# kfjahnke/envutil

Measured on AMD Instinct MI355X. Metric: Mpix/s reprojected (16K lat/lon->cubemap, b-spline-3), higher is better.
Workload: dtype f32

## Files before the change

### envutil_amd/csrc/eu_render5.h

```cpp
#define EU5_WAVES 4
#ifndef EU5_TEXELS
#define EU5_TEXELS 576
#endif
#ifndef EU5_OCC
#define EU5_OCC 4
#endif
#ifndef EU5_UNIT_ROWS
#define EU5_UNIT_ROWS 4
#endif

typedef const __attribute__((address_space(3))) eu4_f4 *eu5_l4ptr;

template <int NCH, int DEG>
__device__ __forceinline__ void eu5_taps(eu_lptr lt, int a, int b, int pitch, const eu_f2 *wx, const eu_f2 *wy,
                                         eu_f2 tx, eu_f2 ty, eu_f2 &rga, eu_f2 &bxa, eu_f2 &rgb, eu_f2 &bxb)
{
  constexpr int order = DEG + 1;
  if constexpr (DEG == 1) {
    const eu_f2 wl0 = 1.0f - tx, wr0 = tx, wl1 = 1.0f - ty, wr1 = ty;
    const eu4_f4 a00 = *(eu5_l4ptr)(lt + a), a01 = *(eu5_l4ptr)(lt + a + 4);
    const eu4_f4 a10 = *(eu5_l4ptr)(lt + a + pitch), a11 = *(eu5_l4ptr)(lt + a + pitch + 4);
    const eu4_f4 b00 = *(eu5_l4ptr)(lt + b), b01 = *(eu5_l4ptr)(lt + b + 4);
    const eu4_f4 b10 = *(eu5_l4ptr)(lt + b + pitch), b11 = *(eu5_l4ptr)(lt + b + pitch + 4);
    {
      const eu_f2 l0 = { wl0.x, wl0.x }, r0 = { wr0.x, wr0.x }, l1 = { wl1.x, wl1.x }, r1 = { wr1.x, wr1.x };
      eu_f2 s = a00.xy * l0; s = s + a01.xy * r0; s = s * l1;
      eu_f2 u = a10.xy * l0; u = u + a11.xy * r0; rga = s + u * r1;
      s = a00.zw * l0; s = s + a01.zw * r0; s = s * l1;
      u = a10.zw * l0; u = u + a11.zw * r0; bxa = s + u * r1;
    }
    {
      const eu_f2 l0 = { wl0.y, wl0.y }, r0 = { wr0.y, wr0.y }, l1 = { wl1.y, wl1.y }, r1 = { wr1.y, wr1.y };
      eu_f2 s = b00.xy * l0; s = s + b01.xy * r0; s = s * l1;
      eu_f2 u = b10.xy * l0; u = u + b11.xy * r0; rgb = s + u * r1;
      s = b00.zw * l0; s = s + b01.zw * r0; s = s * l1;
      u = b10.zw * l0; u = u + b11.zw * r0; bxb = s + u * r1;
    }
  } else {
#pragma unroll
    for (int j = 0; j < order; j++) {
      eu4_f4 ta[order], tb[order];
#pragma unroll
      for (int i = 0; i < order; i++) {
        ta[i] = *(eu5_l4ptr)(lt + a + j * pitch + 4 * i);
        tb[i] = *(eu5_l4ptr)(lt + b + j * pitch + 4 * i);
      }
      const eu_f2 w0a = { wx[0].x, wx[0].x }, w0b = { wx[0].y, wx[0].y };
      eu_f2 ra = ta[0].xy * w0a, qa = ta[0].zw * w0a, rb = tb[0].xy * w0b, qb = tb[0].zw * w0b;
#pragma unroll
      for (int i = 1; i < order; i++) {
        const eu_f2 wa = { wx[i].x, wx[i].x }, wb = { wx[i].y, wx[i].y };
        ra = EU_MAD2(wa, ta[i].xy, ra); qa = EU_MAD2(wa, ta[i].zw, qa);
        rb = EU_MAD2(wb, tb[i].xy, rb); qb = EU_MAD2(wb, tb[i].zw, qb);
      }
      const eu_f2 ya = { wy[j].x, wy[j].x }, yb = { wy[j].y, wy[j].y };
      if (j == 0) { rga = ra * ya; bxa = qa * ya; rgb = rb * yb; bxb = qb * yb; }
      else { rga = EU_MAD2(ra, ya, rga); bxa = EU_MAD2(qa, ya, bxa); rgb = EU_MAD2(rb, yb, rgb); bxb = EU_MAD2(qb, yb, bxb); }
    }
  }
}

__device__ __forceinline__ void eu5_box_reduce(int &q0, int &q1, int &q2, int &q3, int &h0, int &h1, int &h2, int &h3)
{
#define EU5_RED(ctrl)                                        \
  "v_min_i32_dpp %0, %0, %0 " ctrl "\n\t"                    \
  "v_min_i32_dpp %1, %1, %1 " ctrl "\n\t"                    \
  "v_max_i32_dpp %2, %2, %2 " ctrl "\n\t"                    \
  "v_max_i32_dpp %3, %3, %3 " ctrl "\n\t"
  asm("s_nop 1\n\t"
      EU5_RED("row_shr:1 row_mask:0xf bank_mask:0xf")
      EU5_RED("row_shr:2 row_mask:0xf bank_mask:0xf")
      EU5_RED("row_shr:4 row_mask:0xf bank_mask:0xf")
      EU5_RED("row_shr:8 row_mask:0xf bank_mask:0xf")
      "v_mov_b32 %4, %0\n\tv_mov_b32 %5, %1\n\tv_mov_b32 %6, %2\n\tv_mov_b32 %7, %3\n\t"
      "v_min_i32_dpp %4, %0, %4 row_bcast:15 row_mask:0xa bank_mask:0xf\n\t"
      "v_min_i32_dpp %5, %1, %5 row_bcast:15 row_mask:0xa bank_mask:0xf\n\t"
      "v_max_i32_dpp %6, %2, %6 row_bcast:15 row_mask:0xa bank_mask:0xf\n\t"
      "v_max_i32_dpp %7, %3, %7 row_bcast:15 row_mask:0xa bank_mask:0xf\n\t"
      "s_nop 0"
      : "+v"(q0), "+v"(q1), "+v"(q2), "+v"(q3), "=&v"(h0), "=&v"(h1), "=&v"(h2), "=&v"(h3));
#undef EU5_RED
}

struct eu5_box { int mnx, mny, mxx, mxy; };

struct eu5_divtab_t { unsigned v[65]; };
static constexpr eu5_divtab_t eu5_make_divtab()
{
  eu5_divtab_t t = {};
  t.v[0] = 0;
  for (unsigned w = 1; w <= 64; w++) t.v[w] = ((65536u + w - 1) / w) | ((64u / w) << 24);
  return t;
}
__constant__ const eu5_divtab_t eu5_divtab = eu5_make_divtab();

__device__ __forceinline__ eu5_box eu5_box_at(int a, int b, int c, int d, int lane)
{
  eu5_box r;
  r.mnx = __builtin_amdgcn_readlane(a, lane); r.mny = __builtin_amdgcn_readlane(b, lane);
  r.mxx = __builtin_amdgcn_readlane(c, lane); r.mxy = __builtin_amdgcn_readlane(d, lane);
  return r;
}
__device__ __forceinline__ eu5_box eu5_box_join(const eu5_box &a, const eu5_box &b)
{
  eu5_box r = { min(a.mnx, b.mnx), min(a.mny, b.mny), max(a.mxx, b.mxx), max(a.mxy, b.mxy) };
  return r;
}
template <int ORDER>
__device__ __forceinline__ int eu5_box_fits(const eu5_box &b)
{
  if (b.mnx == INT_MAX) return -1;
  const unsigned bw = (unsigned)b.mxx - (unsigned)b.mnx + ORDER, bh = (unsigned)b.mxy - (unsigned)b.mny + ORDER;
  return bw <= 64u && bh <= (unsigned)EU5_TEXELS && bw * bh <= (unsigned)EU5_TEXELS;
}

__device__ __forceinline__ eu_f2 eu5_gate2(eu_f2 c, int kind, float lower, float upper)
{
  if (kind == 0) {
    eu_f2 r = c;
    r = eu_sel2(c < lower, (eu_f2){ lower, lower }, r);
    r = eu_sel2(c > upper, (eu_f2){ upper, upper }, r);
    return r;
  }
  eu_f2 cc = c - lower;
  if (kind == 1) cc = eu_abs2(cc);
  return cc + lower;
}

__device__ __forceinline__ int eu5_out_of_range3(float a, float b, float c)
{
  const float hi = __builtin_fmaxf(__builtin_fmaxf(__builtin_fabsf(a), __builtin_fabsf(b)), __builtin_fabsf(c));
  const float lo = __builtin_fminf(__builtin_fminf(__builtin_fabsf(a), __builtin_fabsf(b)), __builtin_fabsf(c));
  return (hi <= 0x1p40f && lo >= 0x1p-40f) ? 0 : -1;
}

struct eu5_tab8 { eu_f2 c0; float A0, A1, A2, B0, B1, B2; };

template <bool FAST>
__device__ __forceinline__ void eu5_load8(const eu_render_params &p, int tile_y, int x0, int lane, eu5_tab8 &T)
{
  const int pr = lane & 3, rw = (lane >> 2) & 7, hf = lane >> 5;
  const int y = p.row_begin + tile_y * EU4_TH + rw;
  const int yc = y < p.row_end ? y : p.row_end - 1;
  const float *rt = p.row + (long long)(FAST ? yc : eu_frame_row(yc, p.band_shift, p.band_count, p.band_index)) * EU_ROW_FLOATS;
  const int xa = x0 + 8 * hf + 2 * pr, xb = xa + 1;
  const int xac = xa < p.width ? xa : p.width - 1, xbc = xb < p.width ? xb : p.width - 1;
  T.A0 = rt[0]; T.A1 = rt[1]; T.A2 = rt[2]; T.B0 = rt[3]; T.B1 = rt[4]; T.B2 = rt[5];
  T.c0 = (eu_f2){ p.col[xac], p.col[xbc] };
}

struct eu5_co8 {
  eu_f2 tx, ty;
  int ixa, ixb, iya, iyb;
  eu_i2 ok;
};

template <int DEG>
__device__ __forceinline__ void eu5_coords8(const eu_src_dev &s, const float *atab, const eu5_tab8 &T, eu5_co8 &c)
{
  eu_i2 big0 = { 0, 0 }, big1 = { 0, 0 };
  const eu_f2 c0 = T.c0;
  const eu_f2 rx = T.B0 * c0 + T.A0, ry = T.B1 * c0 + T.A1, rz = T.B2 * c0 + T.A2;
  const eu_i2 ok = { ~eu5_out_of_range3(rx.x, ry.x, rz.x), ~eu5_out_of_range3(rx.y, ry.y, rz.y) };
  const eu_f2 q2 = rx * rx + rz * rz;
  const eu_f2 qs = eu_sqrt2_safe(q2);
  const eu_f2 lat = eu_atan2f_2_lean(ry, qs, atab, 1, big0);
  const eu_f2 lon = eu_atan2f_2_lean(rx, rz, atab, 0, big1);
  c.ok = ok & ~(big0 | big1);
  eu_f2 i0 = { (float)((double)lon.x - s.tex_x0), (float)((double)lon.y - s.tex_x0) };
  if (s.cdiv_ok) i0 = eu_div2_const(i0, s.ext_w, s.rcp_ext_w);
  else i0 = eu_div2_rr(i0, s.ext_w, eu_rcp_refined(s.ext_w));
  i0 = i0 * s.total_w; i0 = i0 - .5f;
  const eu_f2 sx = i0 - s.win_x_off;
  const eu_f2 gx = eu5_gate2(sx, s.gate0, s.lower0, s.upper0);
  eu_f2 fx;
  if constexpr (DEG & 1) fx = (eu_f2){ floorf(gx.x), floorf(gx.y) };
  else fx = (eu_f2){ roundf(gx.x), roundf(gx.y) };
  c.tx = gx - fx;
  c.ixa = (int)fx.x; c.ixb = (int)fx.y;
  eu_f2 i1 = { (float)((double)lat.x - s.tex_y0), (float)((double)lat.y - s.tex_y0) };
  if (s.cdiv_ok) i1 = eu_div2_const(i1, s.ext_h, s.rcp_ext_h);
  else i1 = eu_div2_rr(i1, s.ext_h, eu_rcp_refined(s.ext_h));
  i1 = i1 * s.total_h; i1 = i1 - .5f;
  const eu_f2 sy = i1 - s.win_y_off;
  c.ty = eu5_gate2(sy, s.gate1, s.lower1, s.upper1);
}

template <int DEG>
__device__ __forceinline__ void eu5_split_y(eu5_co8 &c)
{
  const eu_f2 gy = c.ty;
  eu_f2 fy;
  if constexpr (DEG & 1) fy = (eu_f2){ floorf(gy.x), floorf(gy.y) };
  else fy = (eu_f2){ roundf(gy.x), roundf(gy.y) };
  c.ty = gy - fy;
  c.iya = (int)fy.x; c.iyb = (int)fy.y;
}

struct eu5_boxes {
  int q0, q1, q2, q3, h0, h1, h2, h3;
  eu5_box full;
  int npass;
  bool clean;
};

template <int DEG, bool GATES>
__device__ __forceinline__ void eu5_box_stage(int gate0, int gate1, float upper0, float upper1, eu_i2 hit, eu_i2 ok,
                                              int ixa, int ixb, int iya, int iyb, eu5_boxes &b)
{
  constexpr int order = DEG + 1;
  int q0 = INT_MAX, q1 = INT_MAX, q2 = INT_MIN, q3 = INT_MIN, h0, h1, h2, h3;
// ... 313 lines not shown
__device__ __forceinline__ void eu5_stage(const eu_src_dev &s, const eu5_box &bx, unsigned lds_tile, int lane)
{
  constexpr int order = DEG + 1;
  const int ibw = bx.mxx - bx.mnx + order, ibh = bx.mxy - bx.mny + order;
  const unsigned tv = eu5_divtab.v[ibw];
  const int k = (int)(tv >> 24);
  const unsigned r = ((unsigned)lane * (tv & 0x1ffffu)) >> 16, c = (unsigned)lane - r * (unsigned)ibw;
  const int bx0 = bx.mnx - DEG / 2, by0 = bx.mny - DEG / 2;
  const unsigned pitchb = (unsigned)(s.es1 * 4);
  const unsigned voff = r * pitchb + c * (NCH * 4u);
  const char *const sb0 = (const char *)(s.base + ((long long)by0 * s.es1 + (long long)bx0 * NCH));
  const unsigned long long step = (unsigned long long)k * pitchb;
  const unsigned dstep = (unsigned)(k * ibw) * 16u;
  if ((int)r < k) {
    const char *sb = sb0;
    unsigned dst = lds_tile;
#pragma unroll 1
    for (int left = ibh; left >= k; left -= k) { eu4_dma_row(dst, voff, sb); sb += step; dst += dstep; }
  }
  if ((int)r < ibh % k) {
    const int full = ibh / k;
    eu4_dma_row(lds_tile + (unsigned)full * dstep, voff, sb0 + (unsigned long long)full * step);
  }
}

#define EU5_BT_RECS 4
#define EU5_BT_WORK 8
#define EU5_WAIT_VM0 0x0F70
typedef unsigned eu5_u3 __attribute__((ext_vector_type(3)));
typedef unsigned eu5_u4 __attribute__((ext_vector_type(4)));
typedef int eu5_i4 __attribute__((ext_vector_type(4)));
typedef const __attribute__((address_space(4))) eu5_i4 *eu5_crec;

__device__ __forceinline__ int eu5_bt_pack(const eu5_box &b, int w3, int c)
{
  if (c == 2) return b.mnx == INT_MAX ? -1 : (int)(((unsigned)b.mxx - (unsigned)b.mnx) | (((unsigned)b.mxy - (unsigned)b.mny) << 16));
  return c == 0 ? b.mnx : c == 1 ? b.mny : w3;
}

template <int DEG>
__global__ __launch_bounds__(256) void eu5_boxplan_kernel(const eu_render_params p, const float *atab_g, const int *l2_rows,
                                                          int tiles16, int ntiles, int *tab)
{
  __shared__ __attribute__((aligned(16))) float atab[768];
  const int lane = threadIdx.x & 63;
  const int wave = __builtin_amdgcn_readfirstlane(threadIdx.x >> 6);
  if (wave == 0) {
#pragma unroll
    for (int i = 0; i < 3; i++)
      __builtin_amdgcn_global_load_lds((eu4_gbl_void)(atab_g + i * 256 + lane * 4), (eu4_lds_void)(atab + i * 256), 16, 0, 0);
    asm volatile("s_waitcnt vmcnt(0)" ::: "memory");
  }
  __syncthreads();
  const int g = (int)blockIdx.x * 4 + wave;
  if (g >= ntiles) return;
  const int slot = g / tiles16, tcol = g - slot * tiles16;
  const int tile_y = __builtin_amdgcn_readfirstlane(l2_rows[slot]);
  const int x0 = tcol * EU4_TW;
  const eu_src_dev &s = p.src;
  const int pr = lane & 3, rw = (lane >> 2) & 7, hf = lane >> 5;
  const int y = p.row_begin + tile_y * EU4_TH + rw;
  const bool yin = y < p.row_end;
  const int xa = x0 + 8 * hf + 2 * pr, xb = xa + 1;
  const bool va = yin && xa < p.width, vb = yin && xb < p.width;
  eu5_tab8 T;
  eu5_load8<true>(p, tile_y, x0, lane, T);
  eu5_co8 c;
  eu5_coords8<DEG>(s, atab, T, c);
  eu5_split_y<DEG>(c);
  const eu_i2 hit = { va ? -1 : 0, vb ? -1 : 0 };
  eu5_boxes B;
  eu5_box_stage<DEG, true>(s.gate0, s.gate1, s.upper0, s.upper1, hit, c.ok, c.ixa, c.ixb, c.iya, c.iyb, B);
  const int cls = (B.npass < 0 || (B.npass > 0 && !B.clean)) ? EU5_BT_WORK : B.npass;
  eu5_box r[EU5_BT_RECS] = { B.full, B.full, B.full, B.full };
  if (B.npass == 2) { r[0] = eu5_box_at(B.h0, B.h1, B.h2, B.h3, 31); r[1] = eu5_box_at(B.h0, B.h1, B.h2, B.h3, 63); }
  if (B.npass == 4) {
#pragma unroll
    for (int k = 0; k < 4; k++) r[k] = eu5_box_at(B.q0, B.q1, B.q2, B.q3, 15 + 16 * k);
  }
  int v = 0;
#pragma unroll
  for (int k = 0; k < EU5_BT_RECS; k++) {
#pragma unroll
    for (int i = 0; i < 4; i++)
      if (lane == 4 * k + i) v = eu5_bt_pack(r[k], k == 0 ? cls : 0, i);
  }
  if (lane < 4 * EU5_BT_RECS) tab[(size_t)g * (4 * EU5_BT_RECS) + lane] = v;
}

template <int NCH, int DEG>
__device__ __forceinline__ void eu5_tile_bt(const eu_render_params &p, const eu4_plan &w, const float *atab, float *wtile,
                                            int tile_y, int x0, int lane, const eu5_tab8 &T, eu5_i4 R, eu5_crec rec,
                                            bool have_n, int ty_n, int x0_n, eu5_tab8 &Tn)
{
  constexpr int order = DEG + 1;
  const eu_src_dev &s = p.src;
#ifdef EU5_STAMPS
  unsigned long long st_[8] = { 0, 0, 0, 0, 0, 0, 0, 0 };
#endif
  EU5_STAMP(0);
  const int cls = R.w;
  if (cls & EU5_BT_WORK) {
    if (lane == 0) {
      const int id = tile_y * w.tiles16 + x0 / EU4_TW;
      const int sh = eu4_shard_of(id);
      const int slot = atomicAdd(p.wl + EU4_WL_SHARD(sh), 1);
      p.wl[EU4_WL_ENTRIES + (size_t)slot * EU4_SHARDS + sh] = id;
    }
    if (have_n) eu5_load8<true>(p, ty_n, x0_n, lane, Tn);
    __builtin_amdgcn_s_waitcnt(EU5_WAIT_VM0);
    return;
  }
  const int npass = cls & 7;
  const unsigned lds_tile = (unsigned)(unsigned long long)(eu4_lds_void)wtile;
  eu5_tab8 Tl = T;
  asm volatile("" : "+v"(Tl.c0), "+v"(Tl.A0), "+v"(Tl.A1), "+v"(Tl.A2), "+v"(Tl.B0), "+v"(Tl.B1), "+v"(Tl.B2));
  eu5_box bx = { R.x, R.y, R.x + (R.z & 0xffff), R.y + (R.z >> 16) };
  bool some = npass > 0 && R.z >= 0;
  if (some) eu5_stage<NCH, DEG>(s, bx, lds_tile, lane);
  const int pr = lane & 3, rw = (lane >> 2) & 7, hf = lane >> 5;
  const int y = p.row_begin + tile_y * EU4_TH + rw;
  const bool yin = y < p.row_end;
  const int xa = x0 + 8 * hf + 2 * pr, xb = xa + 1;
  const bool va = yin && xa < p.width, vb = yin && xb < p.width;
  eu_f2 rga = { 0.0f, 0.0f }, bxa = { 0.0f, 0.0f }, rgb = { 0.0f, 0.0f }, bxb = { 0.0f, 0.0f };
  if (npass > 0) {
    eu5_co8 c;
    eu5_coords8<DEG>(s, atab, Tl, c);
    eu5_split_y<DEG>(c);
#ifdef EU5_STAMPS
    asm volatile("" : : "v"(c.iya), "v"(c.iyb), "v"(c.ixa), "v"(c.ixb));
#endif
    EU5_STAMP(2);
#ifdef EU5_STAMPS
    st_[3] = st_[2];
#endif
    eu_f2 wx[order], wy[order];
    if constexpr (DEG >= 2) {
      eu_weights2<DEG>(s.wm, c.ty, wy);
      eu_weights2<DEG>(s.wm, c.tx, wx);
    }
    const int grp = npass == 1 ? 0 : npass == 2 ? hf : (lane >> 4);
#pragma unroll 1
    for (int pi = 0; pi < npass; pi++) {
      eu5_i4 Rn = { 0, 0, -1, 0 };
      if (pi + 1 < npass) Rn = rec[pi + 1];
      if (some) {
        if (pi > 0) eu5_stage<NCH, DEG>(s, bx, lds_tile, lane);
        const int ibw = bx.mxx - bx.mnx + order;
        const bool mine = grp == pi;
        const int oa = (mine && va) ? ((c.iya - bx.mny) * ibw + (c.ixa - bx.mnx)) * 4 : 0;
        const int ob = (mine && vb) ? ((c.iyb - bx.mny) * ibw + (c.ixb - bx.mnx)) * 4 : 0;
        if (pi == 0) EU5_STAMP(4);
        asm volatile("s_waitcnt vmcnt(0)" ::: "memory");
        if (pi == 0) EU5_STAMP(5);
        if (mine) eu5_taps<NCH, DEG>((eu_lptr)wtile, oa, ob, ibw * 4, wx, wy, c.tx, c.ty, rga, bxa, rgb, bxb);
      }
      bx = (eu5_box){ Rn.x, Rn.y, Rn.x + (Rn.z & 0xffff), Rn.y + (Rn.z >> 16) };
      some = Rn.z >= 0;
    }
  }
#ifdef EU5_STAMPS
  asm volatile("" : : "v"(rga), "v"(bxa), "v"(rgb), "v"(bxb));
#endif
  EU5_STAMP(6);
  float qa[4] = { rga.x, rga.y, bxa.x, bxa.y }, qb[4] = { rgb.x, rgb.y, bxb.x, bxb.y };
  if (have_n) eu5_load8<true>(p, ty_n, x0_n, lane, Tn);
  __builtin_amdgcn_sched_barrier(0);
  {
    float *const base = p.out + (long long)(tile_y * EU4_TH) * p.out_stride + (long long)x0 * NCH;
    const __amdgpu_buffer_rsrc_t rs = __builtin_amdgcn_make_buffer_rsrc(base, 0, 0x80000000u, 0x00027000);
    const unsigned off = ((unsigned)rw * (unsigned)p.out_stride + (unsigned)((8 * hf + 2 * pr) * NCH)) * 4u;
    const unsigned oa = va ? off : 0xfffff000u, ob = vb ? oa + NCH * 4u : 0xfffff000u;
    if constexpr (NCH == 3) {
      __builtin_amdgcn_raw_buffer_store_b96((eu5_u3){ __float_as_uint(qa[0]), __float_as_uint(qa[1]), __float_as_uint(qa[2]) }, rs, (int)oa, 0, 0);
      __builtin_amdgcn_raw_buffer_store_b96((eu5_u3){ __float_as_uint(qb[0]), __float_as_uint(qb[1]), __float_as_uint(qb[2]) }, rs, (int)ob, 0, 0);
    } else {
      __builtin_amdgcn_raw_buffer_store_b128((eu5_u4){ __float_as_uint(qa[0]), __float_as_uint(qa[1]), __float_as_uint(qa[2]), __float_as_uint(qa[3]) }, rs, (int)oa, 0, 0);
      __builtin_amdgcn_raw_buffer_store_b128((eu5_u4){ __float_as_uint(qb[0]), __float_as_uint(qb[1]), __float_as_uint(qb[2]), __float_as_uint(qb[3]) }, rs, (int)ob, 0, 0);
    }
  }
  EU5_STAMP(7);
#ifdef EU5_STAMPS
  if (lane == 0 && w.stamps) {
    unsigned long long *o = w.stamps + ((size_t)tile_y * w.tiles16 + x0 / EU4_TW) * 8;
    st_[1] = (unsigned long long)(npass + 1);
#pragma unroll
    for (int k = 0; k < 8; k++) o[k] = st_[k];
  }
#endif
}

struct eu5_tab16 {
  eu4_f4 a0, a1, b0, b1;
  eu_f2 c0;
  float A1A, B1A, A1B, B1B;
};

__device__ __forceinline__ void eu5_load16(const eu_render_params &p, const float *ct, int tile_y, int x0, int lane, eu5_tab16 &T)
{
  const int pr = lane & 3, rw = (lane >> 2) & 7, hf = lane >> 5;
  const int yA = p.row_begin + tile_y * EU4_TH + rw, yB = yA + EU4_TH;
  const int ycA = yA < p.row_end ? yA : p.row_end - 1, ycB = yB < p.row_end ? yB : p.row_end - 1;
  const float *rtA = p.row + (long long)ycA * EU_ROW_FLOATS, *rtB = p.row + (long long)ycB * EU_ROW_FLOATS;
  const int xa = x0 + 8 * hf + 2 * pr, xb = xa + 1;
  const int xac = xa < p.width ? xa : p.width - 1, xbc = xb < p.width ? xb : p.width - 1;
  const eu4_f4 *ea = (const eu4_f4 *)(ct + (size_t)xac * EU4_COL_FLOATS);
  const eu4_f4 *eb = (const eu4_f4 *)(ct + (size_t)xbc * EU4_COL_FLOATS);
  T.a0 = ea[0]; T.a1 = ea[1]; T.b0 = eb[0]; T.b1 = eb[1];
  T.A1A = rtA[1]; T.B1A = rtA[4]; T.A1B = rtB[1]; T.B1B = rtB[4];
  T.c0 = (eu_f2){ p.col[xac], p.col[xbc] };
}

typedef const __attribute__((address_space(4))) int *eu5_cint;

__device__ __forceinline__ void eu5_load_cols(const float *ct, int xa, int xb, eu5_tab16 &T)
{
  const eu4_f4 *ea = (const eu4_f4 *)(ct + (size_t)xa * EU4_COL_FLOATS);
  const eu4_f4 *eb = (const eu4_f4 *)(ct + (size_t)xb * EU4_COL_FLOATS);
  T.a0 = ea[0]; T.a1 = ea[1]; T.b0 = eb[0]; T.b1 = eb[1];
}

__device__ __forceinline__ void eu5_y_reduce(int &mn, int &mx)
{
#define EU5_RED2(ctrl)                                       \
  "v_min_i32_dpp %0, %0, %0 " ctrl "\n\t"                    \
  "v_max_i32_dpp %1, %1, %1 " ctrl "\n\t"                    \
  "s_nop 1\n\t"
  asm("s_nop 1\n\t"
      EU5_RED2("row_shr:1 row_mask:0xf bank_mask:0xf")
      EU5_RED2("row_shr:2 row_mask:0xf bank_mask:0xf")
      EU5_RED2("row_shr:4 row_mask:0xf bank_mask:0xf")
      EU5_RED2("row_shr:8 row_mask:0xf bank_mask:0xf")
      EU5_RED2("row_bcast:15 row_mask:0xa bank_mask:0xf")
      EU5_RED2("row_bcast:31 row_mask:0xc bank_mask:0xf")
      : "+v"(mn), "+v"(mx));
#undef EU5_RED2
  mn = __builtin_amdgcn_readlane(mn, 63); mx = __builtin_amdgcn_readlane(mx, 63);
}

template <int NCH, int DEG>
__device__ __forceinline__ void eu5_group16(const eu_render_params &p, const eu4_plan &w, const float *atab, float *wtile,
                                            eu5_tab16 &T, eu5_cint ent, int n, int m0, int plan0, int tcol, int lane0,
                                            bool have_n, int m_n, int plan_n, int tcol_n)
{
  constexpr int order = DEG + 1;
  const eu_src_dev &s = p.src;
#ifdef EU5_STAMPS
  unsigned st_[8] = { 0, 0, 0, 0, 0, 0, 0, 0 };
#endif
  EU5_STAMP32(0);
  const eu5_cint xt = (eu5_cint)w.xtab;
  int xmn = xt[2 * (plan0 * w.tiles16 + tcol)], xmx = xt[2 * (plan0 * w.tiles16 + tcol) + 1];
  int iyAa, iyAb, iyBa, iyBb, bad, mny = INT_MAX, mxy = INT_MIN;
  eu_f2 tyA, tyB;
  bool off;
  {
    int lane = lane0;
    asm volatile("" : "+v"(lane));
    const int pr = lane & 3, rw = (lane >> 2) & 7, hf = lane >> 5;
    const int yA = p.row_begin + 2 * m0 * EU4_TH + rw, yB = yA + EU4_TH;
    const bool yinA = yA < p.row_end, yinB = yB < p.row_end;
    const int xa = tcol * EU4_TW + 8 * hf + 2 * pr, xb = xa + 1;
    const bool vxa = xa < p.width, vxb = xb < p.width;
    const eu_f2 c0 = T.c0;
    const eu_f2 ryA = T.B1A * c0 + T.A1A, ryB = T.B1B * c0 + T.A1B;
    const eu_f2 qs = { T.a1.z, T.b1.z };
    eu_i2 bigA = { 0, 0 }, bigB = { 0, 0 };
    bad = eu5_out_of_range3(ryA.x, qs.x, ryB.x) | eu5_out_of_range3(ryA.y, qs.y, ryB.y);
    const eu_f2 latA = eu_atan2f_2_lean(ryA, qs, atab, 1, bigA);
    const eu_f2 latB = eu_atan2f_2_lean(ryB, qs, atab, 1, bigB);
    bad |= bigA.x | bigA.y | bigB.x | bigB.y;
    const float rr = s.cdiv_ok ? 0.0f : __int_as_float(__builtin_amdgcn_readfirstlane(__float_as_int(eu_rcp_refined(s.ext_h))));
    eu_f2 iA = { (float)((double)latA.x - s.tex_y0), (float)((double)latA.y - s.tex_y0) };
    eu_f2 iB = { (float)((double)latB.x - s.tex_y0), (float)((double)latB.y - s.tex_y0) };
    if (s.cdiv_ok) { iA = eu_div2_const(iA, s.ext_h, s.rcp_ext_h); iB = eu_div2_const(iB, s.ext_h, s.rcp_ext_h); }
    else { iA = eu_div2_rr(iA, s.ext_h, rr); iB = eu_div2_rr(iB, s.ext_h, rr); }
    iA = iA * s.total_h; iA = iA - .5f; iB = iB * s.total_h; iB = iB - .5f;
    const eu_f2 gyA = eu5_gate2(iA - s.win_y_off, s.gate1, s.lower1, s.upper1);
    const eu_f2 gyB = eu5_gate2(iB - s.win_y_off, s.gate1, s.lower1, s.upper1);
    eu_f2 fyA, fyB;
    if constexpr (DEG & 1) { fyA = (eu_f2){ floorf(gyA.x), floorf(gyA.y) }; fyB = (eu_f2){ floorf(gyB.x), floorf(gyB.y) }; }
    else { fyA = (eu_f2){ roundf(gyA.x), roundf(gyA.y) }; fyB = (eu_f2){ roundf(gyB.x), roundf(gyB.y) }; }
    tyA = gyA - fyA; tyB = gyB - fyB;
    iyAa = (int)fyA.x; iyAb = (int)fyA.y; iyBa = (int)fyB.x; iyBb = (int)fyB.y;
#ifdef EU5_STAMPS
    asm volatile("" : : "v"(iyAa), "v"(iyAb), "v"(iyBa), "v"(iyBb));
#endif
    EU5_STAMP32(2);
    const bool hAa = yinA && vxa, hAb = yinA && vxb, hBa = yinB && vxa, hBb = yinB && vxb;
    int q1 = INT_MAX, q3 = INT_MIN;
    if (hAa) { q1 = iyAa; q3 = iyAa; }
    if (hAb) { q1 = min(q1, iyAb); q3 = max(q3, iyAb); }
    if (hBa) { q1 = min(q1, iyBa); q3 = max(q3, iyBa); }
    if (hBb) { q1 = min(q1, iyBb); q3 = max(q3, iyBb); }
    eu5_y_reduce(q1, q3);
    mny = q1; mxy = q3;
    off = __ballot(bad != 0 && (hAa || hAb || hBa || hBb)) != 0ull;
  }
  EU5_STAMP32(3);
  int mk = m0, pk = plan0;
#pragma unroll 1
  for (int k = 0; k < n; k++) {
    int lane = lane0;
    asm volatile("" : "+v"(lane));
    const int pr = lane & 3, rw = (lane >> 2) & 7, hf = lane >> 5;
    const bool mir = (pk & EU_SHARE_MIRROR) != 0;
    const int tc = mir ? w.tiles16 - 1 - tcol : tcol;
    int mk_n = 0, pk_n = 0;
    if (k + 1 < n) { mk_n = ent[2 * k + 4]; pk_n = ent[2 * k + 5]; }
#ifdef EU5_STAMPS
    if (k > 0) { EU5_STAMP32(0); st_[2] = st_[0]; st_[3] = st_[0]; }
#endif
    eu5_box bx = { xmn, mny, xmx, mxy };
    bool fast = !off && xmn != INT_MAX && mny != INT_MAX;
    if (fast) {
      const int cw = __builtin_amdgcn_readfirstlane((int)(s.upper0 + 0.5f)), ch = __builtin_amdgcn_readfirstlane((int)(s.upper1 + 0.5f));
      if (s.gate0 == 2 && bx.mnx < 0) fast = false;
      if (s.gate0 != 0 && bx.mxx >= cw - 1) fast = false;
      if (s.gate1 == 2 && bx.mny < 0) fast = false;
      if (s.gate1 != 0 && bx.mxy >= ch - 1) fast = false;
      if (eu5_box_fits<order>(bx) != 1) fast = false;
    }
    const int xl = 8 * hf + 2 * pr;
    const int xa = mir ? p.width - 1 - (tcol * EU4_TW + xl) : tc * EU4_TW + xl, xb = mir ? xa - 1 : xa + 1;
    const int yA = p.row_begin + 2 * mk * EU4_TH + rw, yB = yA + EU4_TH;
    const bool yinA = yA < p.row_end, yinB = yB < p.row_end;
    const int ycA = yinA ? yA : p.row_end - 1, ycB = yinB ? yB : p.row_end - 1;
    const bool vxa = xa < p.width, vxb = xb < p.width;
    const bool hAa = yinA && vxa, hAb = yinA && vxb, hBa = yinB && vxa, hBb = yinB && vxb;
    eu_f2 rga = { 0.0f, 0.0f }, bxa = { 0.0f, 0.0f }, rgb = { 0.0f, 0.0f }, bxb = { 0.0f, 0.0f };
    if (fast) eu5_stage<NCH, DEG>(s, bx, (unsigned)(unsigned long long)(eu4_lds_void)wtile, lane);
    const bool mir_n = (pk_n & EU_SHARE_MIRROR) != 0;
    const int plan_k = pk_n & (EU_SHARE_MIRROR - 1);
    const int tc_k = mir_n ? w.tiles16 - 1 - tcol : tcol;
    int xmn_n = INT_MAX, xmx_n = INT_MIN;
    if (k + 1 < n) { xmn_n = xt[2 * (plan_k * w.tiles16 + tc_k)]; xmx_n = xt[2 * (plan_k * w.tiles16 + tc_k) + 1]; }
    if (fast) {
      eu_f2 wx[order], wyA[order], wyB[order];
      const int ixa = __float_as_int(T.a0.x), ixb = __float_as_int(T.b0.x);
      const eu_f2 tx = { T.a0.y, T.b0.y };
      if constexpr (DEG >= 2) {
        wx[0] = (eu_f2){ T.a0.z, T.b0.z }; wx[1] = (eu_f2){ T.a0.w, T.b0.w }; wx[2] = (eu_f2){ T.a1.x, T.b1.x };
        if constexpr (DEG == 3) wx[3] = (eu_f2){ T.a1.y, T.b1.y };
        eu_weights2<DEG>(s.wm, tyA, wyA); eu_weights2<DEG>(s.wm, tyB, wyB);
      }
      const int ibw = bx.mxx - bx.mnx + order;
      const int oAa = hAa ? ((iyAa - bx.mny) * ibw + (ixa - bx.mnx)) * 4 : 0, oAb = hAb ? ((iyAb - bx.mny) * ibw + (ixb - bx.mnx)) * 4 : 0;
      const int oBa = hBa ? ((iyBa - bx.mny) * ibw + (ixa - bx.mnx)) * 4 : 0, oBb = hBb ? ((iyBb - bx.mny) * ibw + (ixb - bx.mnx)) * 4 : 0;
      asm volatile("s_waitcnt vmcnt(0)" ::: "memory");
      __builtin_amdgcn_sched_barrier(0);
      eu5_taps<NCH, DEG>((eu_lptr)wtile, oAa, oAb, ibw * 4, wx, wyA, tx, tyA, rga, bxa, rgb, bxb);
      asm volatile("" : "+v"(rga), "+v"(bxa), "+v"(rgb), "+v"(bxb));
      {
        float qa[4] = { rga.x, rga.y, bxa.x, bxa.y }, qb[4] = { rgb.x, rgb.y, bxb.x, bxb.y };
        float *const orow = p.out + (long long)(ycA - p.row_begin) * p.out_stride;
        if (hAa) eu_put<NCH>(orow, xa, qa);
        if (hAb) eu_put<NCH>(orow, xb, qb);
      }
      __builtin_amdgcn_sched_barrier(0);
      eu5_taps<NCH, DEG>((eu_lptr)wtile, oBa, oBb, ibw * 4, wx, wyB, tx, tyB, rga, bxa, rgb, bxb);
      asm volatile("" : "+v"(rga), "+v"(bxa), "+v"(rgb), "+v"(bxb));
    } else if (mny != INT_MAX) {
      if (lane < 2) {
        const int id = (2 * mk + lane) * w.tiles16 + tc;
        const int sh = eu4_shard_of(id);
        const int slot = atomicAdd(p.wl + EU4_WL_SHARD(sh), 1);
        p.wl[EU4_WL_ENTRIES + (size_t)slot * EU4_SHARDS + sh] = id;
      }
    }
    if (k + 1 < n) {
      const int xa_n = mir_n ? p.width - 1 - (tcol * EU4_TW + xl) : tcol * EU4_TW + xl, xb_n = mir_n ? xa_n - 1 : xa_n + 1;
      const int xac = xa_n < p.width ? xa_n : p.width - 1, xbc = xb_n < p.width ? xb_n : p.width - 1;
      eu5_load_cols(w.coltab + (size_t)plan_k * p.width * EU4_COL_FLOATS, xac, xbc, T);
    } else if (have_n) {
      eu5_load16(p, w.coltab + (size_t)plan_n * p.width * EU4_COL_FLOATS, 2 * m_n, tcol_n * EU4_TW, lane, T);
    }
    __builtin_amdgcn_sched_barrier(0);
    if (fast) {
      float qa[4] = { rga.x, rga.y, bxa.x, bxa.y }, qb[4] = { rgb.x, rgb.y, bxb.x, bxb.y };
      float *const orow = p.out + (long long)(ycB - p.row_begin) * p.out_stride;
      if (hBa) eu_put<NCH>(orow, xa, qa);
      if (hBb) eu_put<NCH>(orow, xb, qb);
    }
    EU5_STAMP32(7);
#ifdef EU5_STAMPS
    if (fast && lane == 0 && w.stamps) {
      unsigned long long *o = w.stamps + ((size_t)(2 * mk) * w.tiles16 + tc) * 8;
      st_[1] = (k == 0 ? 6ull : 7ull) | 16ull;
#pragma unroll
      for (int q = 0; q < 8; q++) o[q] = q == 1 ? st_[1] : (q == 4 || q == 5) ? 0ull : (unsigned long long)st_[q == 6 ? 7 : q] | (1ull << 32);
    }
#endif
    mk = mk_n; pk = pk_n; xmn = xmn_n; xmx = xmx_n;
  }
}

template <int UNIT>
struct eu5_iter {
  int ul, ry, rx;
  int du, dy, dx;
  int xcd, units, tiles16;
  __device__ __forceinline__ void start(int t0, int K)
  {
    const int per_unit = UNIT * tiles16;
    ul = t0 / per_unit;
    ry = (t0 - ul * per_unit) / tiles16;
    rx = t0 - ul * per_unit - ry * tiles16;
    du = K / per_unit; dy = (K - du * per_unit) / tiles16; dx = K - du * per_unit - dy * tiles16;
  }
  __device__ __forceinline__ void step()
  {
    rx += dx; ry += dy; ul += du;
    if (rx >= tiles16) { rx -= tiles16; ry++; }
    if (ry >= UNIT) { ry -= UNIT; ul++; }
  }
  __device__ __forceinline__ bool done() const { return ul * 8 + xcd >= units; }
  __device__ __forceinline__ int row() const { return (ul * 8 + xcd) * UNIT + ry; }
  __device__ __forceinline__ int col() const
  {
    const unsigned h = ((unsigned)row() * 0x9E3779B1u) >> 16;
    int c = rx + (int)((h * (unsigned)tiles16) >> 16);
    if (c >= tiles16) c -= tiles16;
    return c;
  }
};

__device__ __forceinline__ int eu5_pair_plan(const int *tileplan, int tiles_y, int m)
{
  if (2 * m + 1 >= tiles_y) return -1;
  const eu5_cint tp = (eu5_cint)tileplan;
  const int a = tp[2 * m], b = tp[2 * m + 1];
  return a == b ? a : -1;
}

template <int NCH, int DEG, int PRJ, bool FAST, bool BOXTAB = false>
__global__ __launch_bounds__(64 * EU5_WAVES, EU5_OCC) void eu_render5_kernel(const eu_render_params p, const eu4_plan w)
{
  __shared__ __attribute__((aligned(16))) float tile_all[EU5_WAVES * EU5_TEXELS * 4];
  __shared__ __attribute__((aligned(16))) float atab[768];
  const int lane0 = threadIdx.x & 63;
  const int wave = __builtin_amdgcn_readfirstlane(threadIdx.x >> 6);
  float *const tile = tile_all + wave * (EU5_TEXELS * 4);
  if (PRJ != EU_CUBEMAP && wave == 0) {
#pragma unroll
    for (int i = 0; i < 3; i++)
      __builtin_amdgcn_global_load_lds((eu4_gbl_void)(w.atab_g + i * 256 + lane0 * 4),
                                       (eu4_lds_void)(atab + i * 256), 16, 0, 0);
    asm volatile("s_waitcnt vmcnt(0)" ::: "memory");
  }
  __syncthreads();
#ifdef EU5_STAMPS
  const unsigned long long ws0 = __builtin_amdgcn_s_memtime();
  unsigned long long ws1 = ws0;
#endif
  const int xcd = (int)(blockIdx.x & 7);
  const int K = (int)(gridDim.x >> 3) * EU5_WAVES;
  const int t0 = (int)(blockIdx.x >> 3) * EU5_WAVES + wave;
  constexpr bool PAIRS = FAST && PRJ == EU_SPHERICAL;
  if constexpr (PAIRS) {
    const int n1 = (w.l1_off[xcd + 1] - w.l1_off[xcd]) * w.l1_ecols;
    const eu5_cint ents = (eu5_cint)w.l1_ent + EU_SHARE_ENTRY_INTS * w.l1_off[xcd];
    int pos1 = t0;
    auto seek = [&](eu5_cint &e, int &n, int &m, int &plan, int &tcol) -> bool {
      if (pos1 >= n1) return false;
      const int r = (int)(((unsigned long long)(unsigned)pos1 * w.l1_magic) >> 40);
      e = ents + EU_SHARE_ENTRY_INTS * r;
      n = e[0]; m = e[2]; plan = e[3];
      const unsigned h = ((unsigned)m * 0x9E3779B1u) >> 16;
      int c = pos1 - r * w.l1_ecols + (int)((h * (unsigned)w.l1_ecols) >> 16);
      if (c >= w.l1_ecols) c -= w.l1_ecols;
      tcol = e[1] + c;
      pos1 += K;
      return true;
    };
    eu5_cint e_a = ents, e_n = ents;
    int n_a = 0, m_a = 0, col_a = 0, plan_a = 0, n_n = 0, m_n = 0, col_n = 0, plan_n = 0;
    bool have_a = seek(e_a, n_a, m_a, plan_a, col_a);
    eu5_tab16 T;
    if (have_a) eu5_load16(p, w.coltab + (size_t)plan_a * p.width * EU4_COL_FLOATS, 2 * m_a, col_a * EU4_TW, lane0, T);
#pragma unroll 1
    while (have_a) {
      const bool have_n = seek(e_n, n_n, m_n, plan_n, col_n);
      eu5_group16<NCH, DEG>(p, w, atab, tile, T, e_a, n_a, m_a, plan_a, col_a, lane0, have_n, m_n, have_n ? plan_n : 0, col_n);
      e_a = e_n; n_a = n_n; m_a = m_n; plan_a = plan_n; col_a = col_n; have_a = have_n;
    }
  }
#ifdef EU5_STAMPS
  ws1 = __builtin_amdgcn_s_memtime();
#endif
  eu5_iter<EU5_UNIT_ROWS> it;
  it.xcd = xcd; it.tiles16 = w.tiles16;
  it.units = (p.tiles_y + EU5_UNIT_ROWS - 1) / EU5_UNIT_ROWS;
  it.start(t0, K);
  if constexpr (PAIRS) {
    int *const queue = p.wl + EU4_WL_DYN(xcd);
    const int nbatch = (w.l2_off[xcd + 1] - w.l2_off[xcd]) * w.l2_half;
    const eu5_cint rows2 = (eu5_cint)w.l2_rows + w.l2_off[xcd];
    auto take = [&]() -> int {
      int v = 0;
      if (lane0 == 0) v = atomicAdd(queue, 1);
      return v;
    };
    if constexpr (BOXTAB) {
      static_assert(FAST && PRJ == EU_SPHERICAL, "the box table is that of the FAST lat/lon second loop");
      const eu5_crec bt = (eu5_crec)w.boxtab;
      auto decode = [&](int j, int &ty, int &tcol, int &ti) -> bool {
        if (j >= nbatch) return false;
        const int r = (int)(((unsigned long long)(unsigned)j * w.l2_magic) >> 40);
        ty = rows2[r]; tcol = 2 * (j - r * w.l2_half);
        ti = ((w.l2_off[xcd] + r) * w.tiles16 + tcol) * EU5_BT_RECS;
        return true;
      };
      int ty_a = 0, col_a = 0, ti_a = 0, ty_n = 0, col_n = 0, ti_n = 0;
// ... 86 lines not shown
```

Before: 110,400.

## Software-pipeline LDS tap reads one row-half ahead across both output rows

```diff
diff --git a/envutil_amd/csrc/eu_render5.h b/envutil_amd/csrc/eu_render5.h
--- a/envutil_amd/csrc/eu_render5.h
+++ b/envutil_amd/csrc/eu_render5.h
@@ -11,11 +11,53 @@
 
 typedef const __attribute__((address_space(3))) eu4_f4 *eu5_l4ptr;
 
+template <int DEG> struct eu5_half { eu4_f4 t[DEG + 1]; };
+#define EU5_WAIT_VM0_LGKM0 0x0070
+
+template <int DEG>
+__device__ __forceinline__ void eu5_half_read(eu_lptr lt, int o, eu5_half<DEG> &r)
+{
+#pragma unroll
+  for (int i = 0; i <= DEG; i++) r.t[i] = *(eu5_l4ptr)(lt + o + 4 * i);
+}
+
+template <int NCH, int DEG, bool NEXT>
+__device__ __forceinline__ void eu5_taps_run(eu_lptr lt, int a, int b, int pitch, const eu_f2 *wx, const eu_f2 *wy,
+                                             eu5_half<DEG> &r, int na,
+                                             eu_f2 &rga, eu_f2 &bxa, eu_f2 &rgb, eu_f2 &bxb)
+{
+  constexpr int order = DEG + 1, halves = 2 * order;
+  static_assert(DEG >= 2, "degree 1 reads its four texels at once");
+  eu5_half<DEG> t[2];
+  t[0] = r;
+#pragma unroll
+  for (int h = 0; h < halves; h++) {
+    const int hn = h + 1;
+    if (hn < halves) eu5_half_read<DEG>(lt, ((hn & 1) ? b : a) + (hn >> 1) * pitch, t[hn & 1]);
+    else if (NEXT) eu5_half_read<DEG>(lt, na, t[hn & 1]);
+    const eu4_f4 *const c = t[h & 1].t;
+    if (hn < halves || NEXT) asm volatile("" : "+v"(t[h & 1].t[0]) : : "memory");
+    const int j = h >> 1;
+    const bool pb = (h & 1) != 0;
+    const eu_f2 w0 = pb ? (eu_f2){ wx[0].y, wx[0].y } : (eu_f2){ wx[0].x, wx[0].x };
+    eu_f2 rs = c[0].xy * w0, qs = c[0].zw * w0;
+#pragma unroll
+    for (int i = 1; i < order; i++) {
+      const eu_f2 wi = pb ? (eu_f2){ wx[i].y, wx[i].y } : (eu_f2){ wx[i].x, wx[i].x };
+      rs = EU_MAD2(wi, c[i].xy, rs); qs = EU_MAD2(wi, c[i].zw, qs);
+    }
+    const eu_f2 y = pb ? (eu_f2){ wy[j].y, wy[j].y } : (eu_f2){ wy[j].x, wy[j].x };
+    eu_f2 &rg = pb ? rgb : rga, &bx = pb ? bxb : bxa;
+    if (j == 0) { rg = rs * y; bx = qs * y; }
+    else { rg = EU_MAD2(rs, y, rg); bx = EU_MAD2(qs, y, bx); }
+  }
+  if constexpr (NEXT) r = t[halves & 1];
+}
+
 template <int NCH, int DEG>
 __device__ __forceinline__ void eu5_taps(eu_lptr lt, int a, int b, int pitch, const eu_f2 *wx, const eu_f2 *wy,
                                          eu_f2 tx, eu_f2 ty, eu_f2 &rga, eu_f2 &bxa, eu_f2 &rgb, eu_f2 &bxb)
 {
-  constexpr int order = DEG + 1;
   if constexpr (DEG == 1) {
     const eu_f2 wl0 = 1.0f - tx, wr0 = tx, wl1 = 1.0f - ty, wr1 = ty;
     const eu4_f4 a00 = *(eu5_l4ptr)(lt + a), a01 = *(eu5_l4ptr)(lt + a + 4);
@@ -37,26 +79,9 @@
       u = b10.zw * l0; u = u + b11.zw * r0; bxb = s + u * r1;
     }
   } else {
-#pragma unroll
-    for (int j = 0; j < order; j++) {
-      eu4_f4 ta[order], tb[order];
-#pragma unroll
-      for (int i = 0; i < order; i++) {
-        ta[i] = *(eu5_l4ptr)(lt + a + j * pitch + 4 * i);
-        tb[i] = *(eu5_l4ptr)(lt + b + j * pitch + 4 * i);
-      }
-      const eu_f2 w0a = { wx[0].x, wx[0].x }, w0b = { wx[0].y, wx[0].y };
-      eu_f2 ra = ta[0].xy * w0a, qa = ta[0].zw * w0a, rb = tb[0].xy * w0b, qb = tb[0].zw * w0b;
-#pragma unroll
-      for (int i = 1; i < order; i++) {
-        const eu_f2 wa = { wx[i].x, wx[i].x }, wb = { wx[i].y, wx[i].y };
-        ra = EU_MAD2(wa, ta[i].xy, ra); qa = EU_MAD2(wa, ta[i].zw, qa);
-        rb = EU_MAD2(wb, tb[i].xy, rb); qb = EU_MAD2(wb, tb[i].zw, qb);
-      }
-      const eu_f2 ya = { wy[j].x, wy[j].x }, yb = { wy[j].y, wy[j].y };
-      if (j == 0) { rga = ra * ya; bxa = qa * ya; rgb = rb * yb; bxb = qb * yb; }
-      else { rga = EU_MAD2(ra, ya, rga); bxa = EU_MAD2(qa, ya, bxa); rgb = EU_MAD2(rb, yb, rgb); bxb = EU_MAD2(qb, yb, bxb); }
-    }
+    eu5_half<DEG> r;
+    eu5_half_read<DEG>(lt, a, r);
+    eu5_taps_run<NCH, DEG, false>(lt, a, b, pitch, wx, wy, r, 0, rga, bxa, rgb, bxb);
   }
 }
 
@@ -676,6 +701,7 @@
         const int oa = (mine && va) ? ((c.iya - bx.mny) * ibw + (c.ixa - bx.mnx)) * 4 : 0;
         const int ob = (mine && vb) ? ((c.iyb - bx.mny) * ibw + (c.ixb - bx.mnx)) * 4 : 0;
         if (pi == 0) EU5_STAMP(4);
+        __builtin_amdgcn_s_waitcnt(EU5_WAIT_VM0_LGKM0);
         asm volatile("s_waitcnt vmcnt(0)" ::: "memory");
         if (pi == 0) EU5_STAMP(5);
         if (mine) eu5_taps<NCH, DEG>((eu_lptr)wtile, oa, ob, ibw * 4, wx, wy, c.tx, c.ty, rga, bxa, rgb, bxb);
@@ -867,23 +893,40 @@
       if constexpr (DEG >= 2) {
         wx[0] = (eu_f2){ T.a0.z, T.b0.z }; wx[1] = (eu_f2){ T.a0.w, T.b0.w }; wx[2] = (eu_f2){ T.a1.x, T.b1.x };
         if constexpr (DEG == 3) wx[3] = (eu_f2){ T.a1.y, T.b1.y };
-        eu_weights2<DEG>(s.wm, tyA, wyA); eu_weights2<DEG>(s.wm, tyB, wyB);
+        eu_weights2<DEG>(s.wm, tyA, wyA);
       }
       const int ibw = bx.mxx - bx.mnx + order;
       const int oAa = hAa ? ((iyAa - bx.mny) * ibw + (ixa - bx.mnx)) * 4 : 0, oAb = hAb ? ((iyAb - bx.mny) * ibw + (ixb - bx.mnx)) * 4 : 0;
-      const int oBa = hBa ? ((iyBa - bx.mny) * ibw + (ixa - bx.mnx)) * 4 : 0, oBb = hBb ? ((iyBb - bx.mny) * ibw + (ixb - bx.mnx)) * 4 : 0;
+      __builtin_amdgcn_s_waitcnt(EU5_WAIT_VM0_LGKM0);
       asm volatile("s_waitcnt vmcnt(0)" ::: "memory");
       __builtin_amdgcn_sched_barrier(0);
-      eu5_taps<NCH, DEG>((eu_lptr)wtile, oAa, oAb, ibw * 4, wx, wyA, tx, tyA, rga, bxa, rgb, bxb);
-      asm volatile("" : "+v"(rga), "+v"(bxa), "+v"(rgb), "+v"(bxb));
-      {
-        float qa[4] = { rga.x, rga.y, bxa.x, bxa.y }, qb[4] = { rgb.x, rgb.y, bxb.x, bxb.y };
-        float *const orow = p.out + (long long)(ycA - p.row_begin) * p.out_stride;
-        if (hAa) eu_put<NCH>(orow, xa, qa);
-        if (hAb) eu_put<NCH>(orow, xb, qb);
-      }
-      __builtin_amdgcn_sched_barrier(0);
-      eu5_taps<NCH, DEG>((eu_lptr)wtile, oBa, oBb, ibw * 4, wx, wyB, tx, tyB, rga, bxa, rgb, bxb);
+      if constexpr (DEG >= 2) {
+        eu5_half<DEG> r;
+        eu5_half_read<DEG>((eu_lptr)wtile, oAa, r);
+        const int oBa = hBa ? ((iyBa - bx.mny) * ibw + (ixa - bx.mnx)) * 4 : 0, oBb = hBb ? ((iyBb - bx.mny) * ibw + (ixb - bx.mnx)) * 4 : 0;
+        eu5_taps_run<NCH, DEG, true>((eu_lptr)wtile, oAa, oAb, ibw * 4, wx, wyA, r, oBa, rga, bxa, rgb, bxb);
+        asm volatile("" : "+v"(rga), "+v"(bxa), "+v"(rgb), "+v"(bxb), "+v"(tyB));
+        eu_weights2<DEG>(s.wm, tyB, wyB);
+        {
+          float qa[4] = { rga.x, rga.y, bxa.x, bxa.y }, qb[4] = { rgb.x, rgb.y, bxb.x, bxb.y };
+          float *const orow = p.out + (long long)(ycA - p.row_begin) * p.out_stride;
+          if (hAa) eu_put<NCH>(orow, xa, qa);
+          if (hAb) eu_put<NCH>(orow, xb, qb);
+        }
+        eu5_taps_run<NCH, DEG, false>((eu_lptr)wtile, oBa, oBb, ibw * 4, wx, wyB, r, 0, rga, bxa, rgb, bxb);
+      } else {
+        const int oBa = hBa ? ((iyBa - bx.mny) * ibw + (ixa - bx.mnx)) * 4 : 0, oBb = hBb ? ((iyBb - bx.mny) * ibw + (ixb - bx.mnx)) * 4 : 0;
+        eu5_taps<NCH, DEG>((eu_lptr)wtile, oAa, oAb, ibw * 4, wx, wyA, tx, tyA, rga, bxa, rgb, bxb);
+        asm volatile("" : "+v"(rga), "+v"(bxa), "+v"(rgb), "+v"(bxb));
+        {
+          float qa[4] = { rga.x, rga.y, bxa.x, bxa.y }, qb[4] = { rgb.x, rgb.y, bxb.x, bxb.y };
+          float *const orow = p.out + (long long)(ycA - p.row_begin) * p.out_stride;
+          if (hAa) eu_put<NCH>(orow, xa, qa);
+          if (hAb) eu_put<NCH>(orow, xb, qb);
+        }
+        __builtin_amdgcn_sched_barrier(0);
+        eu5_taps<NCH, DEG>((eu_lptr)wtile, oBa, oBb, ibw * 4, wx, wyB, tx, tyB, rga, bxa, rgb, bxb);
+      }
       asm volatile("" : "+v"(rga), "+v"(bxa), "+v"(rgb), "+v"(bxb));
     } else if (mny != INT_MAX) {
       if (lane < 2) {
```

Result: no change. 110,300 (-0.1%).
